# troyvvgroup/quemb

Hardware: AMD Instinct MI355X
Metric: fragment CCSD iters/sec (full BE sweep over synthetic n_occ=20 n_virt=200 fragments); corr-E error vs oracle in parity_max_abs_err_Eh / parity_n220_abs_err_Eh (higher is better)
Workload: dtype f64

## Files before the change

### include/qemb_hip_ops.h

```cpp
#ifndef QEMB_HIP_OPS_H
#define QEMB_HIP_OPS_H
#include "qemb_hip.h"
#ifdef __cplusplus
extern "C" {
#endif

#define QEMB_TIMER_LADDER 0
#define QEMB_TIMER_RINGS 1
#define QEMB_TIMER_ITER 2
#define QEMB_TIMER_AO2MO 3
#define QEMB_TIMER_SCF 4
#define QEMB_TIMER_GEMM_ANY 5
#define QEMB_TIMER_SCHMIDT 6
#define QEMB_TIMER_DF 7
int qemb_timer_begin(int slot);
int qemb_timer_end(int slot);
int qemb_timer_read(int slot, double* total_ms, int64_t* count);
int qemb_timer_reset(int slot);
int qemb_alloc_stats(long long* n_driver_allocs, long long* n_driver_frees, double* ms_in_driver_calls, double* gb_allocated, int reset);
int qemb_gemm_flop_count(double* flops, int reset);
int qemb_tape_cache_counters(int64_t* reused, int64_t* recorded, int reset);
int qemb_ctx_timer_read(int ctx, int slot, double* total_ms, int64_t* count, int reset);
int qemb_timer_live_events(int slot);

// ... 55 lines not shown
                           const double* OB, const double* OC, double* R, double* W2);
int qemb_op_ccsd_ring_prep_rule(int64_t o, int64_t v, int replay);
int qemb_op_ccsd_u_update(int64_t o, int64_t v, const double* A, const double* t1, const double* Z, double* U);
int qemb_op_copy4_two(const int64_t dim[4], const double* in, const int64_t si[4], double* out, const int64_t so[4], double alpha, double beta, const double* base,
                      double* out2, const double* in2, double c2a, double c2b);
int qemb_op_scatter_pm_rows_add(int64_t o, int64_t ncols, const double* Xp, const double* Xm, double* out, const double* add);
int qemb_op_ccsd_y_traces_add(int64_t o, int64_t v, const double* ZC, const double* ZB, double* Y, const double* add);
int qemb_op_pack_w_pm_sum(int64_t o, const double* Wt, const double* X, const double* At, double* Ap, int64_t lda_p, double* Am, int64_t lda_m);
int qemb_op_ccsd_t1_assemble(int64_t o, int64_t v, const double* t1, const double* Lvv, const double* Loo, const double* Fov, const double* S, const double* Lph1,
                             const double* PA, int SA, int64_t strideA, const double* PB, int SB, int64_t strideB, double* t1n);
int qemb_op_gemv_rows_two(int64_t rows1, int64_t cols1, const double* T1, int64_t ld1, const double* x1, double* y1, double a1, double b1,
                          int64_t rows2, int64_t cols2, const double* T2, int64_t ld2, const double* x2, double* y2, double a2, double b2);
int qemb_op_ccsd_y_traces_slabs(int64_t o, int64_t v, const double* ZC, const double* ZB, double* Y, const double* add, int S, int64_t stride, double scale);
int qemb_op_ccsd_finish_t2_rings(int64_t o, int64_t v, double* t2n, const double* U, const double* OV, const double* RS, const double* M, const double* eo, const double* ev, double* t1n);
int qemb_op_diis_push(int64_t n, const double* trial, const double* prev, double* e, double* xcopy, int m, const double* const* ys, int self, double* row_dev, double* row_host);
int qemb_op_ccsd_extrapolate_energy(int64_t o, int64_t v, int nterms, const double* coef, const double* const* xs, double* amp, const double* L, double* tau, double* e_host);
int qemb_op_gather_rows(int64_t nrows, int64_t len, const int64_t* idx_dev, const double* src, int64_t ld, double* dst);
int qemb_op_scale_rows(int64_t nrows, int64_t len, double* x, const double* s);
int qemb_op_pack_pair_rows(int64_t n, int64_t ncols, const double* in, double* out);
int qemb_op_unpack_tril_pair_rows(int64_t nr, int64_t n, const double* in, double* full);
int qemb_op_extract_pf(int64_t n, const double* Mp, int64_t p0, int64_t q0, int64_t r0, int64_t s0, int64_t sp, int64_t sq,
                       int64_t sr, int64_t ss, double* out);
int qemb_op_extract_pf_t(int64_t n, const double* T, int64_t x0, int64_t r0, int64_t s0, int64_t c0, int64_t sx, int64_t sr,
                         int64_t ss, int64_t sc, double* out);
int qemb_op_ladder_pack_vvvv_pf(int64_t n, int64_t o, const double* Mp, double* Vp, int64_t ldp, double* Vm, int64_t ldm);
int qemb_op_extract_pf_t_compact(int64_t n, const double* T, int64_t x0, int64_t c0, int64_t sx, int64_t sr, int64_t ss, int64_t sc,
                                 double* out, int64_t slab);
int qemb_op_gather_pair_cols(int64_t rows, int64_t n, const double* in, int64_t r0, int64_t s0, int64_t sr, int64_t ss, double* out);
int qemb_op_extract_ps(int64_t n, const double* S, int64_t p0, int64_t q0, int64_t r0, int64_t s0, int64_t sp, int64_t sq,
                       int64_t sr, int64_t ss, double* out);
int qemb_op_extract_ps_packed(int64_t n, const double* S, int64_t p0, int64_t q0, int64_t r0, int64_t sp, int64_t sq, int64_t sr, double* out);
int qemb_op_unpack_pair_block(int64_t n, int64_t o, const double* S, double* Mv, int64_t ld);
int qemb_op_ladder_pack_vvvv_pf_ld(int64_t n, int64_t o, const double* Mp, int64_t ld, double* Vp, int64_t ldp, double* Vm, int64_t ldm);
int qemb_op_pack_pm_ovvv(int64_t o, int64_t v, const double* ovvv, double* Op, int64_t ldp, double* Om, int64_t ldm);
int qemb_op_df_pair_product(int64_t np, int64_t naux, const double* bb, double* out);
int qemb_op_unpack_tril_rows(int64_t rows, int64_t n, const double* packed, double* full);
int qemb_op_pack_tril_rows(int64_t rows, int64_t n, const double* full, double* packed);
int qemb_op_jacobi_eigh(int64_t n, double* A, double* w, double* V, int* sweeps);
int qemb_op_scf_fused_max(void);
int qemb_op_jacobi_eigh_in_basis(int64_t n, const double* F, const double* Cp, double* w, double* C_out, double* C2_out, int nocc, double* dm_out, double stop_below, int* sweeps);
int qemb_op_scf_fock_small(int64_t n, const double* h, const double* J, const double* K, const double* D, double* F, double* err, double* scal2);
int qemb_op_pack_density_sym(int64_t n, const double* D, double* Dp);
int qemb_op_jacobi_svd(int64_t m, int64_t n, double* G, double* s, double* U, double* V, int* sweeps);
int qemb_op_cholesky_lower(int64_t n, double* A);
int qemb_op_tri_inverse_lower(int64_t n, const double* L, double* Linv);


int qemb_op_mp2_amplitudes(int64_t o, int64_t v, const double* ovov, const double* eo, const double* ev, double* t2, double* G, double* e_host);

int qemb_op_rdm2_assemble(int kind, int64_t o, int64_t v, const double* t1, const double* t2, const double* dm1c, double* out);
int qemb_op_ccsd_t(int o, int v, const double* t1, const double* t2, const double* ovvv, const double* ovoo, const double* ovov, const double* eo, const double* ev, int tile, double* e_t);
int qemb_op_rdm2_add_nc(int64_t m, const double* g, double alpha, double* X);
int qemb_op_rdm2_symmetrize(int64_t m, const double* g, double* X);
int qemb_op_rdm2_eri_dot(int64_t m, int sym, const double* eri, const double* K, double* e_host);

int qemb_op_kdf_split(int64_t rows, int64_t nao, const double* z, double* planes);
int qemb_op_kdf_stack(int64_t nk, int64_t nao, int64_t n, const double* ta, double* Cs, double* Dk);
int qemb_op_kdf_pack(int64_t naux, int64_t n, const double* M, int paired, double w, double* F, int64_t ldf, double* out2_host);

int qemb_frag_prepare_ccsd(qemb_frag_t f, int nsocc, const double* h, const double* dm0, const qemb_solver_opts* opts);
int qemb_frag_ccsd_iterate(qemb_frag_t f, int niter, double* e_corr, double* normt);
int qemb_frag_ccsd_reset(qemb_frag_t f);
int qemb_frag_ccsd_export(qemb_frag_t f, const char* name, double* host, int64_t nelem);


int qemb_op_boys(int m_max, int64_t n, const double* x, double* out);
// ... 37 lines not shown
```

### quemb_amd/_lib.py

```python

from __future__ import annotations

import ctypes as C
import os
from pathlib import Path

import numpy as np

_HERE = Path(__file__).resolve().parent
LIB_PATH = _HERE / "libqemb_hip.so"

c_dp = C.POINTER(C.c_double)
c_i64 = C.c_int64
c_vp = C.c_void_p


QEMB_ERR_ARG, QEMB_ERR_ALLOC, QEMB_ERR_DEVICE, QEMB_ERR_NOCONV, QEMB_ERR_NUMERIC, QEMB_ERR_UNSUPPORTED = -1, -2, -3, -4, -5, -6


class QembError(RuntimeError):

    def __init__(self, msg="", status=None):
        super().__init__(msg)
        self.status = status
# ... 96 lines not shown
    f("qemb_op_ccsd_u_update", I, L, L, P, P, P, P)
    f("qemb_op_ccsd_ovvv_slabs", I, L, L)
    f("qemb_op_ccsd_ovvv_pass", I, L, L, P, P, P, P, P)
    f("qemb_op_ccsd_y_traces", I, L, L, P, P, P)
    f("qemb_op_copy4_two", I, C.POINTER(L), P, C.POINTER(L), P, C.POINTER(L), D, D, P, P, P, D, D)
    f("qemb_op_scatter_pm_rows_add", I, L, L, P, P, P, P)
    f("qemb_op_ccsd_y_traces_add", I, L, L, P, P, P, P)
    f("qemb_op_pack_w_pm_sum", I, L, P, P, P, P, L, P, L)
    f("qemb_op_ccsd_t1_assemble", I, L, L, P, P, P, P, P, P, P, I, L, P, I, L, P)
    f("qemb_op_gemv_rows_two", I, L, L, P, L, P, P, D, D, L, L, P, L, P, P, D, D)
    f("qemb_op_ccsd_y_traces_slabs", I, L, L, P, P, P, P, I, L, D)
    f("qemb_op_ccsd_finish_t2_rings", I, L, L, P, P, P, P, P, P, P, P)
    f("qemb_op_diis_push", I, L, P, P, P, P, I, P, I, P, P)
    f("qemb_op_ccsd_extrapolate_energy", I, L, L, I, P, P, P, P, P, P)
    f("qemb_op_gather_rows", I, L, L, P, P, L, P)
    f("qemb_op_scale_rows", I, L, L, P, P)
    f("qemb_ctx_count", I, I)
    f("qemb_ctx_bind", I, I)
    f("qemb_ctx_partition", I, I)
    f("qemb_ctx_timer_read", I, I, I, C.POINTER(C.c_double), C.POINTER(c_i64), I)
    f("qemb_gemm_flop_count", I, C.POINTER(C.c_double), I)
    f("qemb_tape_cache_counters", I, C.POINTER(L), C.POINTER(L), I)
    f("qemb_alloc_stats", I, C.POINTER(C.c_longlong), C.POINTER(C.c_longlong), C.POINTER(C.c_double), C.POINTER(C.c_double), I)
    f("qemb_op_unpack_tril_pair_rows", I, L, L, P, P)
    f("qemb_op_extract_pf", I, L, P, L, L, L, L, L, L, L, L, P)
    f("qemb_op_extract_pf_t", I, L, P, L, L, L, L, L, L, L, L, P)
    f("qemb_op_ladder_pack_vvvv_pf", I, L, L, P, P, L, P, L)
    f("qemb_op_extract_pf_t_compact", I, L, P, L, L, L, L, L, L, P, L)
    f("qemb_op_gather_pair_cols", I, L, L, P, L, L, L, L, P)
    f("qemb_op_extract_ps", I, L, P, L, L, L, L, L, L, L, L, P)
    f("qemb_op_extract_ps_packed", I, L, P, L, L, L, L, L, L, P)
    f("qemb_op_unpack_pair_block", I, L, L, P, P, L)
    f("qemb_op_ladder_pack_vvvv_pf_ld", I, L, L, P, L, P, L, P, L)
    f("qemb_op_pack_pm_ovvv", I, L, L, P, P, L, P, L)
    f("qemb_op_df_pair_product", I, L, L, P, P)
    f("qemb_op_pack_tril_rows", I, L, L, P, P)
    f("qemb_op_jacobi_eigh", I, L, P, P, P, C.POINTER(I))
    f("qemb_op_scf_fused_max", I)
    f("qemb_op_jacobi_eigh_in_basis", I, L, P, P, P, P, P, I, P, D, C.POINTER(I))
    f("qemb_op_scf_fock_small", I, L, P, P, P, P, P, P, P)
    f("qemb_op_pack_density_sym", I, L, P, P)
    f("qemb_op_jacobi_svd", I, L, L, P, P, P, P, C.POINTER(I))
    f("qemb_op_cholesky_lower", I, L, P)
    f("qemb_op_joint_diag", I, L, L, P, P, D, I, C.POINTER(I), C.POINTER(D), C.POINTER(I))
    f("qemb_df_localize_er", I, V, P, I, D, I, P, C.POINTER(I), C.POINTER(D), C.POINTER(D), C.POINTER(I))
    f("qemb_op_joint_diag_bytes", I, L, L, C.POINTER(L), C.POINTER(I))
    f("qemb_op_joint_diag_mem_limit", I, L)
    f("qemb_op_tri_inverse_lower", I, L, P, P)
    f("qemb_comm_unique_id", I, P)
    f("qemb_comm_init", I, I, I, P)
    f("qemb_comm_info", I, C.POINTER(I), C.POINTER(I))
    f("qemb_comm_allreduce", I, P, L, I)
    f("qemb_comm_destroy", I)
    OP = C.POINTER(SolverOpts)
    IP = C.POINTER(I)
    DP = C.POINTER(D)
    f("qemb_default_opts", None, OP)
    f("qemb_frag_create", I, I, I, C.POINTER(c_vp))
    f("qemb_frag_free", I, V)
    f("qemb_frag_set_eri_s4", I, V, P)
    f("qemb_frag_set_eri_s4_dev", I, V, P)
    f("qemb_frag_set_df_factor", I, V, I, P)
    f("qemb_frag_set_df_factor_dev", I, V, I, P)
    f("qemb_frag_mo_route", I, V, I)
    f("qemb_frag_set_df_only", I, V, I, P)
    f("qemb_frag_set_df_only_dev", I, V, I, V)
# ... 213 lines not shown
```

### quemb_amd/csrc/api.cpp

```cpp
#include <cstring>
#include <cstdlib>
#include <vector>
#include <execinfo.h>
#include <signal.h>
#include <unistd.h>
#include "../../include/qemb_hip_ops.h"
#include "dev_ops.h"
#include "ccsd.h"
#include "fragment.h"
#include "ao2mo.h"
#include "kdf.h"
#include "int3c.h"
#include "int4c.h"
#include "cd_core.h"
#include "loc_core.h"
#include "sci_core.h"
#include <algorithm>
#include <cmath>
#include <mutex>
#include <set>

using namespace qemb;
namespace qemb {
int dev_mfma_f64_peak(int iters, int blocks_per_cu, double* tflops);
// ... 258 lines not shown
  int rc = dev_ccsd_extrapolate_energy(o, v, nterms, coef, xs, amp, L, tau, e_dev, (double*)pin);
  if (!rc) rc = dev_sync();
  if (!rc) *e_host = *(double*)pin;
  dev_pinned_free(pin);
  return rc;
}
int qemb_op_ccsd_y_traces(int64_t o, int64_t v, const double* ZC, const double* ZB, double* Y) { return dev_ccsd_y_traces(o, v, ZC, ZB, Y); }
int qemb_op_gather_rows(int64_t nrows, int64_t len, const int64_t* idx_dev, const double* src, int64_t ld, double* dst) { return dev_gather_rows(nrows, len, idx_dev, src, ld, dst); }
int qemb_op_scale_rows(int64_t nrows, int64_t len, double* x, const double* s) { return dev_scale_rows(nrows, len, x, s); }
int qemb_op_pack_pair_rows(int64_t n, int64_t ncols, const double* in, double* out) { return dev_pack_pair_rows(n, ncols, in, out); }
int qemb_op_extract_pf(int64_t n, const double* Mp, int64_t p0, int64_t q0, int64_t r0, int64_t s0, int64_t sp, int64_t sq, int64_t sr, int64_t ss, double* out) {
  return dev_extract_pf(n, Mp, p0, q0, r0, s0, sp, sq, sr, ss, out);
}
int qemb_op_extract_pf_t(int64_t n, const double* T, int64_t x0, int64_t r0, int64_t s0, int64_t c0, int64_t sx, int64_t sr, int64_t ss, int64_t sc, double* out) {
  return dev_extract_pf_t(n, T, x0, r0, s0, c0, sx, sr, ss, sc, out);
}
int qemb_op_ladder_pack_vvvv_pf(int64_t n, int64_t o, const double* Mp, double* Vp, int64_t ldp, double* Vm, int64_t ldm) { return dev_ladder_pack_vvvv_pf(n, o, Mp, Vp, ldp, Vm, ldm); }
int qemb_op_extract_pf_t_compact(int64_t n, const double* T, int64_t x0, int64_t c0, int64_t sx, int64_t sr, int64_t ss, int64_t sc, double* out, int64_t slab) {
  return dev_extract_pf_t_compact(n, T, x0, c0, sx, sr, ss, sc, out, slab);
}
int qemb_op_gather_pair_cols(int64_t rows, int64_t n, const double* in, int64_t r0, int64_t s0, int64_t sr, int64_t ss, double* out) {
  return dev_gather_pair_cols(rows, n, in, r0, s0, sr, ss, out);
}
int qemb_op_extract_ps(int64_t n, const double* S, int64_t p0, int64_t q0, int64_t r0, int64_t s0, int64_t sp, int64_t sq, int64_t sr, int64_t ss, double* out) {
  return dev_extract_ps(n, S, p0, q0, r0, s0, sp, sq, sr, ss, out);
}
int qemb_op_extract_ps_packed(int64_t n, const double* S, int64_t p0, int64_t q0, int64_t r0, int64_t sp, int64_t sq, int64_t sr, double* out) {
  return dev_extract_ps_packed(n, S, p0, q0, r0, sp, sq, sr, out);
}
int qemb_op_unpack_pair_block(int64_t n, int64_t o, const double* S, double* Mv, int64_t ld) { return dev_unpack_pair_block(n, o, S, Mv, ld); }
int qemb_op_ladder_pack_vvvv_pf_ld(int64_t n, int64_t o, const double* Mp, int64_t ld, double* Vp, int64_t ldp, double* Vm, int64_t ldm) {
  return dev_ladder_pack_vvvv_pf_ld(n, o, Mp, ld, Vp, ldp, Vm, ldm);
}
int qemb_op_pack_pm_ovvv(int64_t o, int64_t v, const double* ovvv, double* Op, int64_t ldp, double* Om, int64_t ldm) { return dev_pack_pm_ovvv(o, v, ovvv, Op, ldp, Om, ldm); }
int qemb_op_df_pair_product(int64_t np, int64_t naux, const double* bb, double* out) { return df_pair_product(np, naux, bb, out); }
int qemb_op_unpack_tril_pair_rows(int64_t nr, int64_t n, const double* in, double* full) { return dev_unpack_tril_pair_rows(nr, n, in, full); }
int qemb_op_unpack_tril_rows(int64_t rows, int64_t n, const double* p, double* f) { return dev_unpack_tril_rows(rows, n, p, f); }
int qemb_op_pack_tril_rows(int64_t rows, int64_t n, const double* f, double* p) { return dev_pack_tril_rows(rows, n, f, p); }
int qemb_op_jacobi_eigh(int64_t n, double* A, double* w, double* V, int* sweeps) { return dev_jacobi_eigh(n, A, w, V, sweeps); }
int qemb_op_scf_fused_max(void) { return dev_scf_fused_max(); }
int qemb_op_jacobi_eigh_in_basis(int64_t n, const double* F, const double* Cp, double* w, double* C_out, double* C2_out, int nocc, double* dm_out, double stop_below, int* sweeps) {
  DBuf st;
  QTRY(st.alloc(1));
  QTRY(dev_jacobi_eigh_in_basis(n, F, Cp, w, C_out, C2_out, nocc, dm_out, stop_below, reinterpret_cast<int*>(st.p)));
  double word = 0.0;
  QTRY(dev_d2h(&word, st.p, sizeof(double)));
  int sw; std::memcpy(&sw, &word, sizeof(int));
  if (sweeps) *sweeps = sw;
  return jacobi_status_code(sw, "dev_jacobi_eigh_in_basis");
}
int qemb_op_scf_fock_small(int64_t n, const double* h, const double* J, const double* K, const double* D, double* F, double* err, double* scal2) { return dev_scf_fock_small(n, h, J, K, D, F, err, scal2); }
int qemb_op_pack_density_sym(int64_t n, const double* D, double* Dp) { return dev_pack_density_sym(n, D, Dp); }
int qemb_op_jacobi_svd(int64_t m, int64_t n, double* G, double* s, double* U, double* V, int* sweeps) { return dev_jacobi_svd(m, n, G, s, U, V, sweeps); }
int qemb_op_cholesky_lower(int64_t n, double* A) { return dev_cholesky_lower(n, A); }
static thread_local int64_t g_joint_diag_limit = -1;
int qemb_op_joint_diag_mem_limit(int64_t bytes) { g_joint_diag_limit = bytes; return QEMB_OK; }
int qemb_op_joint_diag_bytes(int64_t K, int64_t m, int64_t* bytes, int* in_lds) {
  if (K < 0 || m < 0 || !bytes) { set_error("qemb_op_joint_diag_bytes: bad arguments"); return QEMB_ERR_ARG; }
  *bytes = (int64_t)loc::footprint_bytes(K, m);
  if (in_lds) *in_lds = loc::in_lds(K, m) ? 1 : 0;
  return QEMB_OK;
}
static int joint_diag_guard(const char* who, int64_t K, int64_t m, double extra_bytes, double to_allocate) {
  size_t free_b = 0, total_b = 0;
  QTRY(dev_mem_info(&free_b, &total_b));
  const double need = loc::footprint_bytes(K, m) + extra_bytes;
// ... 1026 lines not shown
```

### quemb_amd/csrc/ccsd.cpp

```cpp
#include "ccsd.h"
#include "ao2mo.h"
#include <algorithm>
#include <chrono>
#include <cmath>
#include <cstdio>
#include <cstdlib>
#include <cstring>
#include <string>

namespace qemb {

int mo_slab_ld(int n) { return (n >= 64 && n <= 1024) ? (n + 15) / 16 * 16 : n; }
int64_t mo_transform_work(int n) { return (int64_t)n * mo_slab_ld(n) * ((int64_t)n * (n + 1) / 2); }

static int mo_three_quarter_blocks(int n, int o, int nf, const double* T, int64_t slab, MoIntegrals& out, bool build_T34) {
  const int v = n - o;
  if (nf > 0 && build_T34) {
    QTRY(out.T34.alloc((int64_t)n * n * n * nf));
    QTRY(dev_extract_pf_t(n, T, 0, 0, 0, 0, n, n, n, nf, out.T34, slab));
  } else if (nf > 0) {
    QTRY(out.A1.alloc((int64_t)v * o * v * nf));
    QTRY(out.A2.alloc((int64_t)o * o * v * nf));
    QTRY(dev_extract_pf_t(n, T, o, 0, o, 0, v, o, v, nf, out.A1, slab));
    QTRY(dev_extract_pf_t(n, T, 0, 0, o, 0, o, o, v, nf, out.A2, slab));
  }
  return 0;
}

static int mo_three_quarter_blocks_ov(int n, int o, int nf, const double* T, int64_t slab, MoIntegrals& out) {
  const int v = n - o;
  QTRY(out.A1.alloc((int64_t)v * o * v * nf));
  QTRY(out.A2.alloc((int64_t)o * o * v * nf));
  QTRY(dev_extract_pf_t_compact(n, T, o, 0, v, o, v, nf, out.A1, slab));
  QTRY(dev_extract_pf_t_compact(n, T, 0, 0, o, o, v, nf, out.A2, slab));
  return 0;
}

static void packed_pair_lds(int64_t v, int64_t& ldp, int64_t& ldm) {
  const int64_t npv = v * (v + 1) / 2, nm = v * (v - 1) / 2;
  ldp = npv + (npv & 1);
  ldm = nm > 0 ? nm + (nm & 1) : 2;
}

static int mo_blocks_from_pair_product(int n, int o, const double* S, double* work, MoIntegrals& out) {
  const int v = n - o;
  const int64_t npv = (int64_t)v * (v + 1) / 2, nm = (int64_t)v * (v - 1) / 2;
  QTRY(out.oooo.alloc((int64_t)o * o * o * o));
  QTRY(out.ovoo.alloc((int64_t)o * v * o * o));
  QTRY(out.ovov.alloc((int64_t)o * v * o * v));
  QTRY(out.oovv.alloc((int64_t)o * o * v * v));
  QTRY(out.ovvo.alloc((int64_t)o * v * v * o));
  QTRY(out.ovvv.alloc((int64_t)o * v * v * v));
  QTRY(out.ovvv_pk.alloc((int64_t)o * v * npv));
  QTRY(dev_extract_ps(n, S, 0, 0, 0, 0, o, o, o, o, out.oooo));
  QTRY(dev_extract_ps(n, S, 0, o, 0, 0, o, v, o, o, out.ovoo));
  QTRY(dev_extract_ps(n, S, 0, o, 0, o, o, v, o, v, out.ovov));
  QTRY(dev_extract_ps(n, S, 0, 0, o, o, o, o, v, v, out.oovv));
  QTRY(dev_extract_ps(n, S, 0, o, o, 0, o, v, v, o, out.ovvo));
  QTRY(dev_extract_ps_packed(n, S, 0, o, o, o, v, v, out.ovvv_pk));
  QTRY(dev_unpack_tril_rows((int64_t)o * v, v, out.ovvv_pk, out.ovvv));
  packed_pair_lds(v, out.ldp, out.ldm);
  QTRY(out.Vp.alloc(npv * out.ldp));
  QTRY(out.Vm.alloc(std::max<int64_t>(nm, 1) * out.ldm));
  const int64_t ldv = mo_slab_ld(v);
  QTRY(dev_unpack_pair_block(n, o, S, work, ldv));
  QTRY(dev_ladder_pack_vvvv_pf_ld(v, 0, work, ldv, out.Vp, out.ldp, out.Vm, out.ldm));
  return 0;
}

static int mo_blocks_from_pair_first(int n, int o, const double* Mp, double* scratch, int64_t scratch_elems, MoIntegrals& out, bool build_Vl) {
  const int v = n - o;
  QTRY(out.oooo.alloc((int64_t)o * o * o * o));
  QTRY(out.ovoo.alloc((int64_t)o * v * o * o));
  QTRY(out.ovov.alloc((int64_t)o * v * o * v));
  QTRY(out.oovv.alloc((int64_t)o * o * v * v));
  QTRY(out.ovvo.alloc((int64_t)o * v * v * o));
  QTRY(out.ovvv.alloc((int64_t)o * v * v * v));
  QTRY(dev_extract_pf(n, Mp, 0, 0, 0, 0, o, o, o, o, out.oooo));
  QTRY(dev_extract_pf(n, Mp, 0, o, 0, 0, o, v, o, o, out.ovoo));
  QTRY(dev_extract_pf(n, Mp, 0, o, 0, o, o, v, o, v, out.ovov));
  QTRY(dev_extract_pf(n, Mp, 0, 0, o, o, o, o, v, v, out.oovv));
  QTRY(dev_extract_pf(n, Mp, 0, o, o, 0, o, v, v, o, out.ovvo));
  QTRY(dev_extract_pf(n, Mp, 0, o, o, o, o, v, v, v, out.ovvv));
  {
    const int64_t npv = (int64_t)v * (v + 1) / 2, nm = (int64_t)v * (v - 1) / 2;
    packed_pair_lds(v, out.ldp, out.ldm);
    QTRY(out.Vp.alloc(npv * out.ldp));
    QTRY(out.Vm.alloc(std::max<int64_t>(nm, 1) * out.ldm));
    QTRY(dev_ladder_pack_vvvv_pf(n, o, Mp, out.Vp, out.ldp, out.Vm, out.ldm));
  }
  if (build_Vl) {
    const int64_t v4 = (int64_t)v * v * v * v;
    QTRY(out.Vl.alloc(v4));
    DBuf tmp;
    double* g = scratch;
    if (!g || v4 > scratch_elems) { QTRY(tmp.alloc(v4)); g = tmp; }
    QTRY(dev_extract_pf(n, Mp, o, o, o, o, v, v, v, v, g));
    QTRY(perm4(out.Vl, g, v, v, v, v, 0, 2, 1, 3));
  }
// ... 25 lines not shown
    g.C = X0; g.ldc = n; g.strideC = 0; g.batch = 1; g.cfg = GEMM_128x224; g.ksplit = 0;
    QTRY(dev_gemm(g));
  } else QTRY(gemm(n, n, n, 1.0, C, n, false, X1, n, false, 0.0, X0, n, np, 0, n2, n2, tcfg));
  QTRY(mo_blocks_from_pair_first(n, o, X0, X1, mo_transform_work(n), out, build_Vl));
  QTRY(lap_AO2MO.close());
  return 0;
}

int mo_transform_factor(int n, int o, int nf, int naux, const double* Bf, double* X0, double* X1, const double* C, MoIntegrals& out, bool build_Vl,
                        bool build_T34) {
  const int v = n - o;
  const int64_t np = (int64_t)n * (n + 1) / 2, n2 = (int64_t)n * n;
  if (naux <= 0 || !Bf) { set_error("mo_transform_factor: no factor"); return QEMB_ERR_ARG; }
  if ((int64_t)nf * n > mo_transform_work(n) / np) { set_error("mo_transform_factor: work buffer too small"); return QEMB_ERR_ARG; }
  out.n = n; out.o = o; out.v = v; out.nf = nf;
  TimerScope lap_AO2MO(TIMER_AO2MO);
  DBuf Lu, Lh, Lpk;
  QTRY(Lu.alloc((int64_t)naux * n2)); QTRY(Lh.alloc((int64_t)naux * n2)); QTRY(Lpk.alloc((int64_t)naux * np));
  QTRY(dev_unpack_tril_rows(naux, n, Bf, Lu));
  QTRY(gemm((int64_t)naux * n, n, n, 1.0, Lu, n, true, C, n, false, 0.0, Lh, n));
  QTRY(gemm(n, n, n, 1.0, C, n, false, Lh, n, false, 0.0, Lu, n, naux, 0, n2, n2));
  QTRY(dev_pack_tril_rows(naux, n, Lu, Lpk));
  Lu.release();
  QTRY(df_pair_product(np, naux, Lpk, X1));
  if (!build_Vl && !build_T34) {
    if (nf > 0) {
      DBuf Lov;
      QTRY(Lov.alloc((int64_t)naux * o * v));
      QTRY(dev_gather_pair_cols(naux, n, Lpk, 0, o, o, v, Lov));
      QTRY(gemm((int64_t)o * v, (int64_t)nf * n, naux, 1.0, Lov, (int64_t)o * v, false, Lh, n2, false, 0.0, X0, (int64_t)nf * n));
      QTRY(mo_three_quarter_blocks_ov(n, o, nf, X0, (int64_t)nf * n, out));
    }
    Lh.release(); Lpk.release();
    QTRY(mo_blocks_from_pair_product(n, o, X1, X0, out));
    QTRY(lap_AO2MO.close());
    return 0;
  }
  QTRY(dev_unpack_tril_rows(np, n, X1, X0));
  if (nf > 0) {
    QTRY(gemm(np, (int64_t)nf * n, naux, 1.0, Lpk, np, false, Lh, n2, false, 0.0, X1, (int64_t)nf * n));
    QTRY(mo_three_quarter_blocks(n, o, nf, X1, (int64_t)nf * n, out, build_T34));
  }
  Lh.release(); Lpk.release();
  QTRY(mo_blocks_from_pair_first(n, o, X0, X1, mo_transform_work(n), out, build_Vl));
  QTRY(lap_AO2MO.close());
  return 0;
}

static bool use_ovvv_pass(int64_t o, int64_t v, bool replay);
int CcsdSolver::setup(MoIntegrals&& ints, const double* mo_energy_dev) {
  I_ = std::move(ints);
  o_ = I_.o; v_ = I_.v; nf_ = I_.nf;
  const int64_t o = o_, v = v_, nov = o * v, oo = o * o, vv = v * v, N2 = oo * vv;
  QTRY(eo_.alloc(o)); QTRY(ev_.alloc(v));
  QTRY(dev_d2d(eo_, mo_energy_dev, sizeof(double) * o));
  QTRY(dev_d2d(ev_, mo_energy_dev + o, sizeof(double) * v));
  QTRY(ovov_t_.alloc(nov * nov)); QTRY(Lovov_.alloc(nov * nov)); QTRY(Loovv_.alloc(N2)); QTRY(OVoovv_.alloc(N2));
  QTRY(Lovoo_.alloc(o * v * oo)); QTRY(W1base_.alloc(N2)); QTRY(W2base_.alloc(N2)); QTRY(Lph1_.alloc(N2));
  QTRY(oooo_p_.alloc(oo * oo));
  QTRY(perm4(ovov_t_, I_.ovov, o, v, o, v, 0, 3, 2, 1));
  QTRY(dcopy(nov * nov, I_.ovov, Lovov_));
  QTRY(axpby(nov * nov, -1.0, ovov_t_, 2.0, Lovov_));
  QTRY(perm4(Loovv_, Lovov_, o, v, o, v, 0, 2, 1, 3));
  QTRY(perm4(OVoovv_, I_.ovov, o, v, o, v, 0, 2, 1, 3));
  QTRY(perm4(Lovoo_, I_.ovoo, o, v, o, o, 2, 1, 0, 3, -1.0, 0.0));
  QTRY(axpby(o * v * oo, 2.0, I_.ovoo, 1.0, Lovoo_));
  QTRY(LovooT_.alloc(o * v * oo));
// ... 628 lines not shown
```

### quemb_amd/csrc/dev_ops.h

```cpp
#pragma once
#include <cstddef>
#include <cstdint>
#include <string>
#include "../../include/qemb_hip_ops.h"
#include "gemm_tiles.h"
#include "env.h"

namespace qemb {

void set_error(const std::string& msg);
const char* last_error();

#define QTRY(expr)              \
  do {                          \
    int _rc = (expr);           \
    if (_rc != 0) return _rc;   \
  } while (0)


int dev_init(int device);
int dev_sync();
int dev_sync_device();
int dev_ctx_count(int n);
int dev_ctx_bind(int k);
// ... 120 lines not shown
int dev_copy4(const Copy4Desc& c);

struct Outer4Desc {
  int64_t dim[4];
  const double* u; int64_t su0, su2;
  const double* v; int64_t sv1, sv3;
  double* out; int64_t so[4];
  double alpha, beta;
  const double* base = nullptr;
};
int dev_outer4(const Outer4Desc& c);
int dev_lincomb(int64_t n, int nterms, const double* coef, const double* const* xs, double beta, double* out);

int dev_div_denom(double* x, int64_t d0, int64_t d1, int64_t d2, int64_t d3,
                  const double* ea, const double* eb, const double* ec, const double* ed);

int dev_mirror_lower(int64_t n, double* A, int64_t lda);

int dev_k_from_pairs(int64_t n, const double* H, const double* D, double* K);
int dev_jk_from_packed(int64_t n, const double* S4, const double* D, const double* Dp, double* Jp, double* K);

int dev_pack_pair_rows(int64_t n, int64_t ncols, const double* in, double* out);
int dev_extract_pf(int64_t n, const double* Mp, int64_t p0, int64_t q0, int64_t r0, int64_t s0, int64_t sp, int64_t sq,
                   int64_t sr, int64_t ss, double* out);
int dev_extract_pf_t(int64_t n, const double* T, int64_t x0, int64_t r0, int64_t s0, int64_t c0, int64_t sx, int64_t sr,
                     int64_t ss, int64_t sc, double* out, int64_t slab = 0);
int dev_ladder_pack_vvvv_pf(int64_t n, int64_t o, const double* Mp, double* Vp, int64_t ldp, double* Vm, int64_t ldm);
int dev_extract_pf_t_compact(int64_t n, const double* T, int64_t x0, int64_t c0, int64_t sx, int64_t sr, int64_t ss, int64_t sc, double* out, int64_t slab = 0);
int dev_gather_pair_cols(int64_t rows, int64_t n, const double* in, int64_t r0, int64_t s0, int64_t sr, int64_t ss, double* out);
int dev_extract_ps(int64_t n, const double* S, int64_t p0, int64_t q0, int64_t r0, int64_t s0, int64_t sp, int64_t sq, int64_t sr, int64_t ss, double* out);
int dev_extract_ps_packed(int64_t n, const double* S, int64_t p0, int64_t q0, int64_t r0, int64_t sp, int64_t sq, int64_t sr, double* out);
int dev_unpack_pair_block(int64_t n, int64_t o, const double* S, double* Mv, int64_t ld);
int dev_ladder_pack_vvvv_pf_ld(int64_t n, int64_t o, const double* Mp, int64_t ld, double* Vp, int64_t ldp, double* Vm, int64_t ldm);

int dev_ladder_pack_vvvv(int64_t n, int64_t o, const double* M, double* Vp, int64_t ldp, double* Vm, int64_t ldm);
int dev_ladder_pack_tau(int64_t o, int64_t v, const double* tau, double* Tp, int64_t ldp, double* Tm, int64_t ldm);
int dev_pack_pm_cols(int64_t rows, int64_t v, const double* in, double* Op, int64_t ldp, double* Om, int64_t ldm);
int dev_pack_pm_ovvv(int64_t o, int64_t v, const double* ovvv, double* Op, int64_t ldp, double* Om, int64_t ldm);
int dev_scatter_pm_rows(int64_t o, int64_t ncols, const double* Xp, const double* Xm, double* out, const double* add = nullptr, int Sp = 1, int64_t strideP = 0,
                        int Sm = 1, int64_t strideM = 0);
int dev_ccsd_finish_t2_rings(int64_t o, int64_t v, double* t2n, const double* U, const double* OV, const double* RS, const double* M, const double* eo, const double* ev, double* t1n);
int dev_ladder_scatter_pm(int64_t o, int64_t v, const double* Rp, int64_t ldp, const double* Rm, int64_t ldm, double* t2);
int dev_ladder_scatter_pm2(int64_t o, int64_t v, const double* Rp, int64_t ldp, const double* Rm, int64_t ldm, const double* Hp, const double* Hm,
                           int assign, double* t2, int Sp = 1, int64_t strideP = 0, int Sm = 1, int64_t strideM = 0, int64_t ldhp = 0, int64_t ldhm = 0);
int dev_pack_w_pm(int64_t o, const double* W, double* Ap, int64_t lda_p, double* Am, int64_t lda_m);
int dev_pack_w_pm_sum(int64_t o, const double* Wt, const double* X, const double* At, double* Ap, int64_t lda_p, double* Am, int64_t lda_m);
int dev_ccsd_t1_assemble(int64_t o, int64_t v, const double* t1, const double* Lvv, const double* Loo, const double* Fov, const double* S, const double* Lph1,
                         const double* PA, int SA, int64_t strideA, const double* PB, int SB, int64_t strideB, double* t1n);
int dev_gemv_rows_two(int64_t rows1, int64_t cols1, const double* T1, int64_t ld1, const double* x1, double* y1, double a1, double b1,
                      int64_t rows2, int64_t cols2, const double* T2, int64_t ld2, const double* x2, double* y2, double a2, double b2);
int dev_foo_from_x(int64_t o, const double* X, double* F);
int dev_ccsd_ph_layouts(int64_t o, int64_t v, const double* t2, const double* t1, double* T, double* Tp, double* S, double* Ut, double* Tpt, double* Th);
int dev_ccsd_ph_layouts_ring(int64_t o, int64_t v, const double* t2, const double* t1, double* Tp, double* S, double* Ut, double* Tpt);
constexpr int CCSD_OVVV_MAX_TILES = 48;
constexpr int CCSD_OVVV_MAX_ROWT = 18;
inline bool ccsd_ovvv_shape_ok(int64_t o, int64_t v) {
  if (o < 1 || v < 1 || o > 32) return false;
  const int64_t rt = (v + 15) / 16, nt = (2 * o + 15) / 16;
  return rt * nt <= CCSD_OVVV_MAX_TILES && rt + nt <= CCSD_OVVV_MAX_ROWT;
}
int dev_ccsd_ovvv_slabs(int64_t o, int64_t v);
int dev_ccsd_ovvv_pass(int64_t o, int64_t v, const double* ovvv, const double* t1, const double* Thk, double* ZB, double* PA);
constexpr int CCSD_RING_PREP_MAX_O = 32;
inline bool ccsd_ring_prep_shape_ok(int64_t o, int64_t v) { return o >= 1 && o <= CCSD_RING_PREP_MAX_O && v >= 1 && v <= 4096; }
int dev_ccsd_ring_prep(int64_t o, int64_t v, const double* t1, const double* P1, const double* W1base, const double* W2base, const double* ZB, const double* ZC,
                       const double* OB, const double* OC, double* R, double* W2);
// ... 172 lines not shown
```

### quemb_amd/csrc/dev_ops_hip.hip

```cpp
#include <hip/hip_runtime.h>
#include <chrono>
#include <atomic>
#include <algorithm>
#include <cstdint>
#include <cstdlib>
#include <cstring>
#include <map>
#include <thread>
#include <mutex>
#include <string>
#include <type_traits>
#include <vector>
#include "dev_ops.h"
#include "hip_common.h"
#include "grouped_launch.h"

namespace qemb {
static thread_local std::string g_err;
void set_error(const std::string& msg) { g_err = msg; }
const char* last_error() { return g_err.c_str(); }

struct TimerLap { hipEvent_t e0, e1; bool ended; };
struct TimerSlot { double total_ms = 0; int64_t count = 0; std::vector<TimerLap> pending; std::vector<std::pair<hipEvent_t, hipEvent_t>> spare; };
static constexpr size_t TIMER_MAX_PENDING = 64;
// ... 1518 lines not shown
    double* vm = (a > b) ? Vm + (a * (a - 1) / 2 + b) * ldm : nullptr;
    for (long long cd0 = threadIdx.x; cd0 < ldp; cd0 += 4 * (long long)blockDim.x) {
      double x[4], y[4]; long long cc[4], dd[4]; bool in[4];
#pragma unroll
      for (int u = 0; u < 4; ++u) {
        const long long cd = cd0 + u * (long long)blockDim.x;
        in[u] = cd < np;
        long long c = 0, d = 0;
        if (in[u]) unpair_ge(cd, c, d);
        cc[u] = c; dd[u] = d;
        x[u] = in[u] ? Mp[pair_idx(o + a, o + c) * n2 + (o + b) * ld + (o + d)] : 0.0;
        y[u] = in[u] ? Mp[pair_idx(o + b, o + c) * n2 + (o + a) * ld + (o + d)] : 0.0;
      }
#pragma unroll
      for (int u = 0; u < 4; ++u) {
        const long long cd = cd0 + u * (long long)blockDim.x;
        if (cd >= ldp) continue;
        if (!in[u]) { vp[cd] = 0.0; continue; }
        vp[cd] = x[u] + y[u];
        if (vm && cc[u] > dd[u]) vm[cc[u] * (cc[u] - 1) / 2 + dd[u]] = x[u] - y[u];
      }
    }
    if (vm) for (long long q = nm + threadIdx.x; q < ldm; q += blockDim.x) vm[q] = 0.0;
  }
}
int dev_ladder_pack_vvvv_pf_ld(int64_t n, int64_t o, const double* Mp, int64_t ld, double* Vp, int64_t ldp, double* Vm, int64_t ldm) {
  REQUIRE_INIT();
  const long long v = n - o, np = v * (v + 1) / 2;
  if (np <= 0) return QEMB_OK;
  if (ld < n) { set_error("dev_ladder_pack_vvvv_pf_ld: ld < n"); return QEMB_ERR_ARG; }
  return launch("dev_ladder_pack_vvvv_pf", ladder_pack_vvvv_pf_kernel, dim3((unsigned)std::min<long long>(np, 1 << 20)), dim3(256), 0, g_stream, n, o, Mp, (long long)ld, Vp, ldp, Vm, ldm);
}
int dev_ladder_pack_vvvv_pf(int64_t n, int64_t o, const double* Mp, double* Vp, int64_t ldp, double* Vm, int64_t ldm) { return dev_ladder_pack_vvvv_pf_ld(n, o, Mp, n, Vp, ldp, Vm, ldm); }

__global__ void __launch_bounds__(256) ladder_pack_vvvv_kernel(long long n, long long o, const double* __restrict__ M,
                                                              double* __restrict__ Vp, long long ldp, double* __restrict__ Vm, long long ldm) {
  const long long v = n - o, np = v * (v + 1) / 2;
  for (long long ab = blockIdx.x; ab < np; ab += gridDim.x) {
    long long a, b; unpair_ge(ab, a, b);
    const double* Ma = M + ((o + a) * n) * n * n + (o + b) * n;
    double* vp = Vp + ab * ldp;
    double* vm = (a > b) ? Vm + (a * (a - 1) / 2 + b) * ldm : nullptr;
    for (long long cd = threadIdx.x; cd < ldp; cd += blockDim.x) {
      if (cd >= np) { vp[cd] = 0.0; continue; }
      long long c, d; unpair_ge(cd, c, d);
      const double x = Ma[(o + c) * n * n + (o + d)], y = Ma[(o + d) * n * n + (o + c)];
      vp[cd] = x + y;
      if (vm && c > d) vm[c * (c - 1) / 2 + d] = x - y;
    }
    if (vm) { const long long nm = v * (v - 1) / 2; for (long long q = nm + threadIdx.x; q < ldm; q += blockDim.x) vm[q] = 0.0; }
  }
}
int dev_ladder_pack_vvvv(int64_t n, int64_t o, const double* M, double* Vp, int64_t ldp, double* Vm, int64_t ldm) {
  REQUIRE_INIT();
  const long long v = n - o, np = v * (v + 1) / 2;
  if (np <= 0) return QEMB_OK;
  return launch("dev_ladder_pack_vvvv", ladder_pack_vvvv_kernel, dim3((unsigned)std::min<long long>(np, 1 << 20)), dim3(256), 0, g_stream, n, o, M, Vp, ldp, Vm, ldm);
}
template <int MODE>
__global__ void __launch_bounds__(256) pack_pm_tiled_kernel(long long rows, long long o, long long v, const double* __restrict__ in, double* __restrict__ Op,
                                                            long long ldp, double* __restrict__ Om, long long ldm) {
  __shared__ double tB[32][33];
  const long long np = v * (v + 1) / 2, nm = v * (v - 1) / 2;
  const uint3 LB = xcd_logical_block(block_id(), grid_dim());
  long long tc, td; unpair_ge((long long)LB.x, tc, td);
  const int tx = threadIdx.x & 31, ty = threadIdx.x >> 5;
// ... 1320 lines not shown
```

### quemb_amd/csrc/mo_blocks_ops_hostcheck.cpp

```cpp
#ifdef QEMB_HOSTCHECK
#include <algorithm>
#include "dev_ops.h"

namespace qemb {

static inline int64_t pidx(int64_t i, int64_t j) { return i >= j ? i * (i + 1) / 2 + j : j * (j + 1) / 2 + i; }

int dev_extract_pf_t_compact(int64_t n, const double* T, int64_t x0, int64_t c0, int64_t sx, int64_t sr, int64_t ss, int64_t sc, double* out, int64_t slab) {
  if (slab <= 0) slab = n * n;
  for (int64_t x = 0; x < sx; ++x) for (int64_t r = 0; r < sr; ++r) for (int64_t s = 0; s < ss; ++s) for (int64_t c = 0; c < sc; ++c)
    out[((x * sr + r) * ss + s) * sc + c] = T[(r * ss + s) * slab + (c0 + c) * n + (x0 + x)];
  return 0;
}
int dev_gather_pair_cols(int64_t rows, int64_t n, const double* in, int64_t r0, int64_t s0, int64_t sr, int64_t ss, double* out) {
  const int64_t np = n * (n + 1) / 2;
  for (int64_t L = 0; L < rows; ++L) for (int64_t r = 0; r < sr; ++r) for (int64_t s = 0; s < ss; ++s) out[(L * sr + r) * ss + s] = in[L * np + pidx(r0 + r, s0 + s)];
  return 0;
}
int dev_extract_ps(int64_t n, const double* S, int64_t p0, int64_t q0, int64_t r0, int64_t s0, int64_t sp, int64_t sq, int64_t sr, int64_t ss, double* out) {
  const int64_t np = n * (n + 1) / 2;
  for (int64_t p = 0; p < sp; ++p) for (int64_t q = 0; q < sq; ++q) for (int64_t r = 0; r < sr; ++r) for (int64_t s = 0; s < ss; ++s)
    out[((p * sq + q) * sr + r) * ss + s] = S[pidx(p0 + p, q0 + q) * np + pidx(r0 + r, s0 + s)];
  return 0;
}
int dev_extract_ps_packed(int64_t n, const double* S, int64_t p0, int64_t q0, int64_t r0, int64_t sp, int64_t sq, int64_t sr, double* out) {
  const int64_t np = n * (n + 1) / 2, npr = sr * (sr + 1) / 2;
  for (int64_t p = 0; p < sp; ++p) for (int64_t q = 0; q < sq; ++q) for (int64_t r = 0; r < sr; ++r) for (int64_t s = 0; s <= r; ++s)
    out[(p * sq + q) * npr + pidx(r, s)] = S[pidx(p0 + p, q0 + q) * np + pidx(r0 + r, r0 + s)];
  return 0;
}
int dev_unpack_pair_block(int64_t n, int64_t o, const double* S, double* Mv, int64_t ld) {
  const int64_t v = n - o, np = n * (n + 1) / 2;
  for (int64_t a = 0; a < v; ++a) for (int64_t c = 0; c <= a; ++c) for (int64_t b = 0; b < v; ++b) for (int64_t d = 0; d < v; ++d)
    Mv[(pidx(a, c) * v + b) * ld + d] = S[pidx(o + a, o + c) * np + pidx(o + b, o + d)];
  return 0;
}
int dev_ladder_pack_vvvv_pf_ld(int64_t n, int64_t o, const double* Mp, int64_t ld, double* Vp, int64_t ldp, double* Vm, int64_t ldm) {
  const int64_t v = n - o;
  for (int64_t a = 0; a < v; ++a) for (int64_t b = 0; b <= a; ++b) {
    double* vp = Vp + (a * (a + 1) / 2 + b) * ldp; std::fill(vp, vp + ldp, 0.0);
    double* vm = a > b ? Vm + (a * (a - 1) / 2 + b) * ldm : nullptr; if (vm) std::fill(vm, vm + ldm, 0.0);
    for (int64_t c = 0; c < v; ++c) for (int64_t d = 0; d <= c; ++d) {
      const double x = Mp[(pidx(o + a, o + c) * n + (o + b)) * ld + (o + d)], y = Mp[(pidx(o + b, o + c) * n + (o + a)) * ld + (o + d)];
      vp[c * (c + 1) / 2 + d] = x + y;
      if (vm && c > d) vm[c * (c - 1) / 2 + d] = x - y;
    }
  }
  return 0;
}
int dev_pack_pm_ovvv(int64_t o, int64_t v, const double* in, double* Op, int64_t ldp, double* Om, int64_t ldm) {
  if (v < 32) { set_error("dev_pack_pm_ovvv: tiled pass only (v >= 32)"); return QEMB_ERR_ARG; }
  for (int64_t k = 0; k < o; ++k) for (int64_t a = 0; a < v; ++a) {
    double* tp = Op + (k * v + a) * ldp; std::fill(tp, tp + ldp, 0.0);
    double* tm = Om + (k * v + a) * ldm; std::fill(tm, tm + ldm, 0.0);
    for (int64_t c = 0; c < v; ++c) for (int64_t d = 0; d <= c; ++d) {
      const double x = in[((k * v + d) * v + a) * v + c], y = in[((k * v + c) * v + a) * v + d];
      tp[c * (c + 1) / 2 + d] = x + y;
      if (c > d) tm[c * (c - 1) / 2 + d] = x - y;
    }
  }
  return 0;
}

}
#endif
```

Baseline: 58.98.

## Fuse vvvv unpack and ladder packing into one kernel reading packed pair product

Replaces the two-step path (unpack the virtual pair block of S into a dense work slab, then pack it into symmetric/antisymmetric ladder Vp/Vm) with a single kernel that reads the pair-packed S directly. The kernel exploits Vp/Vm symmetry, writing each element and its transpose through a shared-memory tile, and maps blocks to XCDs in an interleaved order. This removes a large intermediate write/read of the vvvv slab in AO2MO. The cost is scattered reads from packed S and a more complex indexing scheme with 32-bit pair offsets.

After: 59.34, median of 6. Within noise of the previous version (+0.6%).

```diff
diff --git a/include/qemb_hip_ops.h b/include/qemb_hip_ops.h
--- a/include/qemb_hip_ops.h
+++ b/include/qemb_hip_ops.h
@@ -111,6 +111,7 @@
 int qemb_op_extract_ps_packed(int64_t n, const double* S, int64_t p0, int64_t q0, int64_t r0, int64_t sp, int64_t sq, int64_t sr, double* out);
 int qemb_op_unpack_pair_block(int64_t n, int64_t o, const double* S, double* Mv, int64_t ld);
 int qemb_op_ladder_pack_vvvv_pf_ld(int64_t n, int64_t o, const double* Mp, int64_t ld, double* Vp, int64_t ldp, double* Vm, int64_t ldm);
+int qemb_op_ladder_pack_vvvv_ps(int64_t n, int64_t o, const double* S, double* Vp, int64_t ldp, double* Vm, int64_t ldm);
 int qemb_op_pack_pm_ovvv(int64_t o, int64_t v, const double* ovvv, double* Op, int64_t ldp, double* Om, int64_t ldm);
 int qemb_op_df_pair_product(int64_t np, int64_t naux, const double* bb, double* out);
 int qemb_op_unpack_tril_rows(int64_t rows, int64_t n, const double* packed, double* full);
diff --git a/quemb_amd/_lib.py b/quemb_amd/_lib.py
--- a/quemb_amd/_lib.py
+++ b/quemb_amd/_lib.py
@@ -152,6 +152,7 @@
     f("qemb_op_extract_ps_packed", I, L, P, L, L, L, L, L, L, P)
     f("qemb_op_unpack_pair_block", I, L, L, P, P, L)
     f("qemb_op_ladder_pack_vvvv_pf_ld", I, L, L, P, L, P, L, P, L)
+    f("qemb_op_ladder_pack_vvvv_ps", I, L, L, P, P, L, P, L)
     f("qemb_op_pack_pm_ovvv", I, L, L, P, P, L, P, L)
     f("qemb_op_df_pair_product", I, L, L, P, P)
     f("qemb_op_pack_tril_rows", I, L, L, P, P)
diff --git a/quemb_amd/csrc/api.cpp b/quemb_amd/csrc/api.cpp
--- a/quemb_amd/csrc/api.cpp
+++ b/quemb_amd/csrc/api.cpp
@@ -314,6 +314,9 @@
 int qemb_op_ladder_pack_vvvv_pf_ld(int64_t n, int64_t o, const double* Mp, int64_t ld, double* Vp, int64_t ldp, double* Vm, int64_t ldm) {
   return dev_ladder_pack_vvvv_pf_ld(n, o, Mp, ld, Vp, ldp, Vm, ldm);
 }
+int qemb_op_ladder_pack_vvvv_ps(int64_t n, int64_t o, const double* S, double* Vp, int64_t ldp, double* Vm, int64_t ldm) {
+  return dev_ladder_pack_vvvv_ps(n, o, S, Vp, ldp, Vm, ldm);
+}
 int qemb_op_pack_pm_ovvv(int64_t o, int64_t v, const double* ovvv, double* Op, int64_t ldp, double* Om, int64_t ldm) { return dev_pack_pm_ovvv(o, v, ovvv, Op, ldp, Om, ldm); }
 int qemb_op_df_pair_product(int64_t np, int64_t naux, const double* bb, double* out) { return df_pair_product(np, naux, bb, out); }
 int qemb_op_unpack_tril_pair_rows(int64_t nr, int64_t n, const double* in, double* full) { return dev_unpack_tril_pair_rows(nr, n, in, full); }
diff --git a/quemb_amd/csrc/ccsd.cpp b/quemb_amd/csrc/ccsd.cpp
--- a/quemb_amd/csrc/ccsd.cpp
+++ b/quemb_amd/csrc/ccsd.cpp
@@ -42,7 +42,7 @@
   ldm = nm > 0 ? nm + (nm & 1) : 2;
 }
 
-static int mo_blocks_from_pair_product(int n, int o, const double* S, double* work, MoIntegrals& out) {
+static int mo_blocks_from_pair_product(int n, int o, const double* S, MoIntegrals& out) {
   const int v = n - o;
   const int64_t npv = (int64_t)v * (v + 1) / 2, nm = (int64_t)v * (v - 1) / 2;
   QTRY(out.oooo.alloc((int64_t)o * o * o * o));
@@ -62,9 +62,7 @@
   packed_pair_lds(v, out.ldp, out.ldm);
   QTRY(out.Vp.alloc(npv * out.ldp));
   QTRY(out.Vm.alloc(std::max<int64_t>(nm, 1) * out.ldm));
-  const int64_t ldv = mo_slab_ld(v);
-  QTRY(dev_unpack_pair_block(n, o, S, work, ldv));
-  QTRY(dev_ladder_pack_vvvv_pf_ld(v, 0, work, ldv, out.Vp, out.ldp, out.Vm, out.ldm));
+  QTRY(dev_ladder_pack_vvvv_ps(n, o, S, out.Vp, out.ldp, out.Vm, out.ldm));
   return 0;
 }
 
@@ -156,7 +154,7 @@
       QTRY(mo_three_quarter_blocks_ov(n, o, nf, X0, (int64_t)nf * n, out));
     }
     Lh.release(); Lpk.release();
-    QTRY(mo_blocks_from_pair_product(n, o, X1, X0, out));
+    QTRY(mo_blocks_from_pair_product(n, o, X1, out));
     QTRY(lap_AO2MO.close());
     return 0;
   }
diff --git a/quemb_amd/csrc/dev_ops.h b/quemb_amd/csrc/dev_ops.h
--- a/quemb_amd/csrc/dev_ops.h
+++ b/quemb_amd/csrc/dev_ops.h
@@ -176,6 +176,7 @@
 int dev_extract_ps_packed(int64_t n, const double* S, int64_t p0, int64_t q0, int64_t r0, int64_t sp, int64_t sq, int64_t sr, double* out);
 int dev_unpack_pair_block(int64_t n, int64_t o, const double* S, double* Mv, int64_t ld);
 int dev_ladder_pack_vvvv_pf_ld(int64_t n, int64_t o, const double* Mp, int64_t ld, double* Vp, int64_t ldp, double* Vm, int64_t ldm);
+int dev_ladder_pack_vvvv_ps(int64_t n, int64_t o, const double* S, double* Vp, int64_t ldp, double* Vm, int64_t ldm);
 
 int dev_ladder_pack_vvvv(int64_t n, int64_t o, const double* M, double* Vp, int64_t ldp, double* Vm, int64_t ldm);
 int dev_ladder_pack_tau(int64_t o, int64_t v, const double* tau, double* Tp, int64_t ldp, double* Tm, int64_t ldm);
diff --git a/quemb_amd/csrc/dev_ops_hip.hip b/quemb_amd/csrc/dev_ops_hip.hip
--- a/quemb_amd/csrc/dev_ops_hip.hip
+++ b/quemb_amd/csrc/dev_ops_hip.hip
@@ -1574,6 +1574,77 @@
   return launch("dev_ladder_pack_vvvv_pf", ladder_pack_vvvv_pf_kernel, dim3((unsigned)std::min<long long>(np, 1 << 20)), dim3(256), 0, g_stream, n, o, Mp, (long long)ld, Vp, ldp, Vm, ldm);
 }
 int dev_ladder_pack_vvvv_pf(int64_t n, int64_t o, const double* Mp, double* Vp, int64_t ldp, double* Vm, int64_t ldm) { return dev_ladder_pack_vvvv_pf_ld(n, o, Mp, n, Vp, ldp, Vm, ldm); }
+__global__ void __launch_bounds__(256) ladder_pack_vvvv_ps_kernel(long long n, long long o, const double* __restrict__ S, double* __restrict__ Vp, long long ldp,
+                                                                 double* __restrict__ Vm, long long ldm) {
+  __shared__ double tp[32][33], tm[32][33];
+  const int v = (int)(n - o), oi = (int)o;
+  const long long npn = n * (n + 1) / 2;
+  const int xcd = blockIdx.x & 7, k = blockIdx.x >> 3;
+  const int aj = k / v, c = k - aj * v;
+  const int a = v - 1 - (aj * 8 + ((aj & 1) ? 7 - xcd : xcd));
+  if (a < 0) return;
+  const int tx = threadIdx.x & 31, ty = threadIdx.x >> 5;
+  const int va = oi + a, vc = oi + c;
+  const double* __restrict__ xrow = S + pair_idx(va, vc) * npn + oi;
+  const double* __restrict__ ycol = S + (long long)va * (va + 1) / 2 + oi;
+  const long long pa = (long long)a * (a + 1) / 2, pc = (long long)c * (c + 1) / 2, qa = (long long)a * (a - 1) / 2, qc = (long long)c * (c - 1) / 2;
+  if (c == 0) {
+    const long long npv = (long long)v * (v + 1) / 2, nm = (long long)v * (v - 1) / 2, wp = ldp - npv, wm = ldm - nm;
+    for (long long t = threadIdx.x; t < (a + 1) * wp; t += blockDim.x) Vp[(pa + t / wp) * ldp + npv + t % wp] = 0.0;
+    for (long long t = threadIdx.x; t < a * wm; t += blockDim.x) Vm[(qa + t / wm) * ldm + nm + t % wm] = 0.0;
+  }
+  const int tbn = a / 32 + 1, tdc = c / 32;
+  int tb = 0, td = 0;
+  while (tb < tbn) {
+    const int b0 = tb * 32 + ty, d = td * 32 + tx;
+    double x[4], y[4];
+#pragma unroll
+    for (int i = 0; i < 4; ++i) {
+      const int b = b0 + 8 * i, vb = oi + b;
+      const bool in = b <= a && d <= b && d <= c;
+      x[i] = in ? xrow[vb * (vb + 1) / 2 + d] : 0.0;
+      y[i] = in ? ycol[pair_idx(vb, vc) * npn + d] : 0.0;
+    }
+    {
+      double* __restrict__ vp = Vp + (pa + b0) * ldp + pc + d;
+      double* __restrict__ vm = Vm + (qa + b0) * ldm + qc + d;
+#pragma unroll
+      for (int i = 0; i < 4; ++i) {
+        const int b = b0 + 8 * i;
+        const double p = x[i] + y[i], m = x[i] - y[i];
+        tp[ty + 8 * i][tx] = p;
+        tm[ty + 8 * i][tx] = m;
+        if (!(b <= a && d <= b && d <= c)) continue;
+        vp[i * 8 * ldp] = p;
+        if (a > b && c > d) vm[i * 8 * ldm] = m;
+      }
+    }
+    __syncthreads();
+    {
+      const int b = tb * 32 + tx, d0 = td * 32 + ty;
+      double* __restrict__ vp = Vp + (pc + d0) * ldp + pa + b;
+      double* __restrict__ vm = Vm + (qc + d0) * ldm + qa + b;
+#pragma unroll
+      for (int i = 0; i < 4; ++i) {
+        const int dm = d0 + 8 * i;
+        if (!(b <= a && dm < b && dm <= c)) continue;
+        vp[i * 8 * ldp] = tp[tx][ty + 8 * i];
+        if (a > b && c > dm) vm[i * 8 * ldm] = tm[tx][ty + 8 * i];
+      }
+    }
+    __syncthreads();
+    if (++td > (tb < tdc ? tb : tdc)) { td = 0; ++tb; }
+  }
+}
+int dev_ladder_pack_vvvv_ps(int64_t n, int64_t o, const double* S, double* Vp, int64_t ldp, double* Vm, int64_t ldm) {
+  REQUIRE_INIT();
+  const long long v = n - o, npv = v * (v + 1) / 2, nm = v * (v - 1) / 2;
+  if (npv <= 0) return QEMB_OK;
+  if (o < 0 || ldp < npv || ldm < nm) { set_error("dev_ladder_pack_vvvv_ps: need 0 <= o < n, ldp >= npair(v) and ldm >= v (v - 1) / 2"); return QEMB_ERR_ARG; }
+  const long long groups = (v + 7) / 8 * 8 * v;
+  if (n > 32768) { set_error("dev_ladder_pack_vvvv_ps: n too large (pair offsets inside a row of S are 32-bit)"); return QEMB_ERR_ARG; }
+  return launch("dev_ladder_pack_vvvv_ps", ladder_pack_vvvv_ps_kernel, dim3((unsigned)groups), dim3(256), 0, g_stream, n, o, S, Vp, ldp, Vm, ldm);
+}
 
 __global__ void __launch_bounds__(256) ladder_pack_vvvv_kernel(long long n, long long o, const double* __restrict__ M,
                                                               double* __restrict__ Vp, long long ldp, double* __restrict__ Vm, long long ldm) {
diff --git a/quemb_amd/csrc/mo_blocks_ops_hostcheck.cpp b/quemb_amd/csrc/mo_blocks_ops_hostcheck.cpp
--- a/quemb_amd/csrc/mo_blocks_ops_hostcheck.cpp
+++ b/quemb_amd/csrc/mo_blocks_ops_hostcheck.cpp
@@ -48,6 +48,25 @@
   }
   return 0;
 }
+int dev_ladder_pack_vvvv_ps(int64_t n, int64_t o, const double* S, double* Vp, int64_t ldp, double* Vm, int64_t ldm) {
+  const int64_t v = n - o, np = n * (n + 1) / 2, npv = v * (v + 1) / 2, nm = v * (v - 1) / 2;
+  if (npv <= 0) return 0;
+  if (o < 0 || ldp < npv || ldm < nm) { set_error("dev_ladder_pack_vvvv_ps: need 0 <= o < n, ldp >= npair(v) and ldm >= v (v - 1) / 2"); return QEMB_ERR_ARG; }
+  for (int64_t ab = 0; ab < npv; ++ab) std::fill(Vp + ab * ldp + npv, Vp + (ab + 1) * ldp, 0.0);
+  for (int64_t ab = 0; ab < nm; ++ab) std::fill(Vm + ab * ldm + nm, Vm + (ab + 1) * ldm, 0.0);
+  for (int64_t a = 0; a < v; ++a) for (int64_t c = 0; c < v; ++c) for (int64_t b = 0; b <= a; ++b) for (int64_t d = 0; d <= std::min(b, c); ++d) {
+    const double x = S[pidx(o + a, o + c) * np + pidx(o + b, o + d)], y = S[pidx(o + b, o + c) * np + pidx(o + a, o + d)];
+    const int64_t pab = a * (a + 1) / 2 + b, pcd = c * (c + 1) / 2 + d, qab = a * (a - 1) / 2 + b, qcd = c * (c - 1) / 2 + d;
+    const bool minus = a > b && c > d;
+    Vp[pab * ldp + pcd] = x + y;
+    if (minus) Vm[qab * ldm + qcd] = x - y;
+    if (d < b) {
+      Vp[pcd * ldp + pab] = x + y;
+      if (minus) Vm[qcd * ldm + qab] = x - y;
+    }
+  }
+  return 0;
+}
 int dev_pack_pm_ovvv(int64_t o, int64_t v, const double* in, double* Op, int64_t ldp, double* Om, int64_t ldm) {
   if (v < 32) { set_error("dev_pack_pm_ovvv: tiled pass only (v >= 32)"); return QEMB_ERR_ARG; }
   for (int64_t k = 0; k < o; ++k) for (int64_t a = 0; a < v; ++a) {
```
